# privacy-scaling-explorations/zkevm-specs

Hardware: AMD Instinct MI355X
Metric: BN254 constraint-rows/sec (higher is better)
Workload: dtype u256 (BN254 Fr: 4xu64 canonical cells, u32-limb Montgomery); 1 GPU; EVM circuit, 2^18 execution steps per GPU, mixed-opcode synthetic trace (BASELINE configs[2]); RW table 816377 rows, bytecode table 43913 rows; steps_per_gpu=262144, rw_rows=816377, bytecode_rows=43913, witness_copies=3

## Files before the change

### zkevm_specs_amd/csrc/evm_circuit.hpp

```cpp
#pragma once
#include "common.hpp"
#include "evm_tables.h"
#include "keccak.hpp"
#include "secp_constants.h"
#include "bigz.hpp"

enum { S_STATE = 0, S_RWC, S_CALL_ID, S_IS_ROOT, S_IS_CREATE, S_CH_LO, S_CH_HI, S_PC, S_SP, S_GAS, S_MWS, S_REV, S_LOG, STEP_NCELLS };
enum { R_RWC = 0, R_RW, R_TAG, R_ID, R_ADDR, R_FT, R_KEY_LO, R_KEY_HI, R_VAL_LO, R_VAL_HI, R_PREV_LO, R_PREV_HI, R_AUX_LO, R_AUX_HI, RW_NCELLS };
enum { B_HASH_LO = 0, B_HASH_HI, B_TAG, B_INDEX, B_IS_CODE, B_VALUE, BYTECODE_NCELLS };
enum { TX_NCELLS = 5, BLOCK_NCELLS = 4 };
enum { CT_IS_FIRST = 0, CT_SRC_ID_LO, CT_SRC_ID_HI, CT_SRC_TAG, CT_DST_ID_LO, CT_DST_ID_HI, CT_DST_TAG, CT_SRC_ADDR,
       CT_SRC_ADDR_END, CT_DST_ADDR, CT_LENGTH, CT_RLC_ACC, CT_RWC, CT_RWC_INC, COPY_T_NCELLS };
enum { XT_IS_STEP = 0, XT_ID, XT_IS_LAST, XT_BASE0, XT_BASE1, XT_BASE2, XT_BASE3, XT_EXP_LO, XT_EXP_HI, XT_RES_LO, XT_RES_HI,
       EXP_T_NCELLS };
enum { SIG_T_NCELLS = 9, ECC_T_NCELLS = 13 };
enum { AUX_PAIR = 3, AUX_ECRECOVER = 5, AUX_ECADD = 6, AUX_ECMUL = 7, AUX_ECPAIRING = 8 };
enum { CDT_Bytecode = 1, CDT_Memory, CDT_TxCalldata, CDT_TxLog, CDT_RlcAcc };

struct EvmDyn {
    u32 rw_sparse;
    u32 codes_n;
    u64 rw_base;
    u32 codes_mask;
    u32 agg_max_txs, agg_total_txs, agg_invalid_txs, agg_bad_invalid_rows, agg_total_wds;
    u32 dir_entries;
    u32 n_deferred;
    u32 agg_rw_dups;
};

struct EvmArgs {
    const EvmDyn* dyn;
    const u64* steps;
    const u32* step_recs;
    u64 n_steps;
    ZkTable rw, bytecode, tx, block;
    ZkTable copy, keccak, exp;
    ZkTable sig, ecc;
    ZkTable withdrawals;
    u32 agg_max_txs, agg_total_txs, agg_invalid_txs, agg_bad_invalid_rows, agg_total_wds;
    u32 agg_rw_dups;
    const u64* aux;
    const u32* aux_kind;
    u32 aux_cells;
    u32 rw_dense;
    u64 rw_base;
    const u64* rw_keys;
    ZkCodeDir codes;
    unsigned long long* prof;
    u32* defer_list;
    u32* defer_count;
    const u32* perm;
    u32 n_pairs;
    u32 opts;
    u32* defer_count_twin;
};

ZK_HD void evm_args_resolve(EvmArgs& a) {
#ifdef EVM_RESOLVE_OFF
    return;
#endif
    if (a.dyn) {
        const EvmDyn d = *a.dyn;
        a.rw_dense = (a.rw.n != 0u && d.rw_sparse == 0u) ? 1u : 0u;
        a.rw_base = d.rw_base;
        a.codes.n = d.codes_n;
        a.codes.mask = d.codes_mask;
        a.agg_max_txs = d.agg_max_txs; a.agg_total_txs = d.agg_total_txs; a.agg_invalid_txs = d.agg_invalid_txs;
        a.agg_bad_invalid_rows = d.agg_bad_invalid_rows; a.agg_total_wds = d.agg_total_wds;
        a.agg_rw_dups = d.agg_rw_dups;
    }
}

#ifndef EVM_HOT_BLOCK
#define EVM_HOT_BLOCK 128
#endif
#define EVM_STAGE_LANES EVM_HOT_BLOCK
#define EV_PROF_WAVE ((blockIdx.x * blockDim.x + threadIdx.x) >> 6)
#define EV_PROF_ON(a) ((a).prof && (threadIdx.x & 63) == 0 && EV_PROF_WAVE < 4096u)
#define EVM_STAGE_STRIDE (EVM_STAGE_LANES + 1)
#define EVM_STAGE_ENTRIES 40
#define EVM_STAGE_GAS 10
ZK_HD constexpr int evm_stage_entry(int s, int c) {
    return c == S_CH_LO || c == S_CH_HI ? 24 + s * 8 + (c - S_CH_LO) * 4
           : s * 12 + (c < S_CH_LO ? c : c == S_PC ? 5 : c == S_SP ? 6 : c == S_MWS ? 7 : c == S_REV ? 8 : c == S_LOG ? 9 : EVM_STAGE_GAS);
}
#define EVM_DIR_MAX_SLOTS 128
#define EVM_DIR_MAX_ENTRIES 32
#define EVM_DIR_SLOT_U64 (EVM_DIR_MAX_SLOTS / 2)
#define EVM_DIR_LDS_U64 (EVM_DIR_SLOT_U64 + EVM_DIR_MAX_ENTRIES * 12)
#if defined(ZK_HOSTSIM)
typedef const u64* EVM_LDS_PTR;
typedef const u32* EVM_LDS32_PTR;
#else
typedef const __attribute__((address_space(3))) u64* EVM_LDS_PTR;
typedef const __attribute__((address_space(3))) u32* EVM_LDS32_PTR;
#endif

struct Word {
    Fr lo, hi;
};
struct WordOrValue {
    Word w;
    bool is_word;
};

#ifndef EVM_FAST
#define EVM_FAST 0
#endif
struct Ins {
    const EvmArgs* a;
    u32 defer;
    u64 idx;
    u32 err;
    u32 seq;
    u64 rw_off;
    u32 pc_off;
    int sp_off;
    Fr rwc, call_id, sp, pc;
    u32 code_state, code_header_row, code_byte_base, code_n_bytes, code_header_ok;
    u64 code_header_value;
    EVM_LDS32_PTR stage;
    EVM_LDS_PTR dir_lds;
    u32 pre_op;
    bool pre_op_ok;
    u32 op_info, op_info_byte;
};

#if defined(ZK_HOSTSIM)
#define EV_PROF(I, k) do { } while (0)
#else
#define EV_PROF(I, k) do { if (EV_PROF_ON(*(I).a)) (I).a->prof[EV_PROF_WAVE * 8 + (k)] = __builtin_readcyclecounter(); } while (0)
#endif

ZK_HD void ev_fail(Ins& I, u32 kind) {
    if (I.err == 0u) I.err = ZK_CODE(kind, I.seq);
}
ZK_HD void ev_require(Ins& I, bool cond, u32 kind = ZK_ASSERT) {
    I.seq++;
    const u32 take = (cond ? 0u : 1u) & (I.err == 0u ? 1u : 0u);
    I.err = take ? ZK_CODE(kind, I.seq) : I.err;
}
#define EV_TRY(stmt) do { stmt; if (I.err) return; } while (0)
#define EV_TRYV(stmt, ret) do { stmt; if (I.err) return ret; } while (0)

ZK_HD Fr ev_step_cell(const EvmArgs& a, u64 step, int c) { return fr_load(a.steps + (step * STEP_NCELLS + c) * 4); }
ZK_HD Fr ev_staged_cell(const Ins& I, int s, int c) {
    Fr r = fr_zero();
    const int e = evm_stage_entry(s, c);
    const int n = (c == S_CH_LO || c == S_CH_HI) ? 4 : c == S_GAS ? 2 : 1;
#pragma unroll
    for (int w = 0; w < n; w++) r.v[w] = I.stage[(e + w) * EVM_STAGE_STRIDE];
    return r;
// ... 4326 lines not shown
```

### zkevm_specs_amd/csrc/evm_kernel.hpp

```cpp
#pragma once
#include "kernels.hpp"

#ifndef ZK_HOT_OCC
#define ZK_HOT_OCC 2
#endif
template <int G, int OCC, int BLOCK>
__global__ __launch_bounds__(BLOCK, OCC) void evm_steps_kernel(EvmArgs a, const u32* group_start, u32* status, ZkTally* tally) {
    u32 perm_t = 0;
    if (G == EVM_GROUP_ALL && a.perm) perm_t = a.perm[(u64)blockIdx.x * blockDim.x + threadIdx.x];
    if (G == EVM_GROUP_ALL && a.defer_count_twin != nullptr) {
        if (blockIdx.x == 0 && threadIdx.x == 0) *a.defer_count_twin = 0u;
        tally_clear_twin(tally);
    }
    __shared__ u64 s_dir[G == EVM_GROUP_ALL ? EVM_DIR_LDS_U64 : 1];
    const bool have_dir = G == EVM_GROUP_ALL && a.dyn != nullptr && a.codes.slots != nullptr && a.codes.entries != nullptr;
    if (have_dir) {
        for (u32 k = threadIdx.x; k < EVM_DIR_SLOT_U64; k += blockDim.x) s_dir[k] = (u64)a.codes.slots[2 * k] | ((u64)a.codes.slots[2 * k + 1] << 32);
        const u64* e = (const u64*)a.codes.entries;
        for (u32 k = threadIdx.x; k < EVM_DIR_MAX_ENTRIES * 12u; k += blockDim.x) s_dir[EVM_DIR_SLOT_U64 + k] = e[k];
    }
    evm_args_resolve(a);
    u32 lo = 0, hi = a.n_pairs;
    if (a.perm) {
        if (G == EVM_GROUP_ALL) hi = group_start[EVM_GROUP_WARM];
        else { lo = group_start[G]; hi = group_start[G + 1]; }
    }
    u64 t = (u64)lo + (u64)blockIdx.x * blockDim.x + threadIdx.x;
    const bool staged_launch = G == EVM_GROUP_ALL || (G == EVM_GROUP_WARM && BLOCK == EVM_HOT_BLOCK && a.perm != nullptr);
    __shared__ u32 s_stage[(G == EVM_GROUP_ALL || (G == EVM_GROUP_WARM && BLOCK == EVM_HOT_BLOCK)) ? EVM_STAGE_ENTRIES * EVM_STAGE_STRIDE : 1];
    if (staged_launch) {
      for (u32 vblock = blockIdx.x;; vblock += gridDim.x) {
        t = (u64)lo + (u64)vblock * blockDim.x + threadIdx.x;
        if ((u64)lo + (u64)vblock * blockDim.x >= (u64)hi) return;
        if (G != EVM_GROUP_ALL && vblock != blockIdx.x) __syncthreads();
        if (G != EVM_GROUP_ALL) perm_t = t < (u64)hi ? a.perm[t] : 0u;
        if (G == EVM_GROUP_ALL && EV_PROF_ON(a)) {
            a.prof[EV_PROF_WAVE * 8 + 5] = __builtin_readcyclecounter();
            a.prof[EV_PROF_WAVE * 8 + 6] = __builtin_amdgcn_s_memrealtime();
        }
        const bool dir_in_lds = have_dir && a.codes.n != 0 && a.codes.n <= EVM_DIR_MAX_ENTRIES && a.codes.mask < EVM_DIR_MAX_SLOTS;
        u32 code = 0;
        u64 idx = t;
        if (t < (u64)hi && a.perm) idx = perm_t;
        const bool mine = t < (u64)hi && idx != (u64)EVM_NO_PAIR;
        __attribute__((address_space(3))) u32* my = (__attribute__((address_space(3))) u32*)s_stage + threadIdx.x;
        const bool wide = a.step_recs ? evm_stage_steps_quad(a, (u32)idx, mine, my - (threadIdx.x & 63u))
                                      : evm_stage_steps_rows_quad(a, (u32)idx, mine, my - (threadIdx.x & 63u));
        if (dir_in_lds) __syncthreads();
        if (mine) {
#if EVM_FAST
            code = wide ? (u32)ZK_DEFERRED_BASE + 8u
                        : evm_check_step<G>(a, idx, (EVM_LDS32_PTR)my, dir_in_lds ? (EVM_LDS_PTR)(__attribute__((address_space(3))) u64*)s_dir : (EVM_LDS_PTR) nullptr);
            if (code >= ZK_DEFERRED_BASE && code != ZK_NOT_MINE) {
#ifdef ZK_DEFER_DEBUG
                if (a.prof) atomicAdd(&a.prof[4095 * 8 - 16 + (code & 15u)], 1ull);
#endif
                a.defer_list[atomicAdd(a.defer_count, 1u)] = (u32)idx;
                code = 0;
            } else
#else
#ifdef ZK_WARM_TWICE
            if (G == EVM_GROUP_WARM)
                code = evm_check_step<G>(a, idx, wide ? (EVM_LDS32_PTR) nullptr : (EVM_LDS32_PTR)my, (EVM_LDS_PTR) nullptr);
#endif
            code = evm_check_step<G>(a, idx, wide ? (EVM_LDS32_PTR) nullptr : (EVM_LDS32_PTR)my,
                                     dir_in_lds ? (EVM_LDS_PTR)(__attribute__((address_space(3))) u64*)s_dir : (EVM_LDS_PTR) nullptr);
#endif
            if (code == ZK_NOT_MINE) code = 0;
            else if (status) status[idx] = code;
        }
        tally_commit(tally, idx, code);
        if (G == EVM_GROUP_ALL && EV_PROF_ON(a)) a.prof[EV_PROF_WAVE * 8 + 7] = __builtin_amdgcn_s_memrealtime();
        if (G == EVM_GROUP_ALL) return;
      }
    } else {
        const u64 stride = (u64)gridDim.x * blockDim.x;
        for (; t < (u64)hi; t += stride) {
            const u64 idx = a.perm ? (u64)a.perm[t] : t;
            u32 code = idx == (u64)EVM_NO_PAIR ? (u32)ZK_NOT_MINE : evm_check_step<G>(a, idx);
            if (code == ZK_NOT_MINE) code = 0;
            else if (status) status[idx] = code;
            tally_commit(tally, idx, code);
        }
    }
}

#if defined(EVM_DEFERRED_KERNEL)
__global__ __launch_bounds__(256, 1) void evm_deferred_kernel(EvmArgs a, u32* status, ZkTally* tally) {
    evm_args_resolve(a);
    const u32 n_def = *a.defer_count;
    const u64 stride = (u64)gridDim.x * blockDim.x;
    for (u64 k = (u64)blockIdx.x * blockDim.x + threadIdx.x; k < (u64)n_def; k += stride) {
        const u64 idx = a.defer_list[k];
        u32 code = evm_check_step<EVM_GROUP_ALL>(a, idx);
        if (code == ZK_NOT_MINE) code = 0;
        else if (status) status[idx] = code;
        tally_commit(tally, idx, code);
    }
}
#endif
```

### zkevm_specs_amd/csrc/zkevm_hip.hip

```cpp
#include <hip/hip_runtime.h>
#include <hip/hip_ext.h>
#include <stdio.h>
#include <string.h>
#include <stdlib.h>
#include <chrono>
#include <string>
#include <vector>

#include <atomic>
#include <mutex>
#include <dlfcn.h>

#include "../../include/zkevm_hip.h"
#include "kernels.hpp"
#include "dist_tally.hpp"
#include "host_index.hpp"
#include "code_dir_build.hpp"

#define ZK_MAX_DEVICES 64
#define ZK_ECDSA_CHUNK_LANES (1ull << 17)
static std::mutex g_dev_mutex;
static hipStream_t g_own_stream[ZK_MAX_DEVICES] = {nullptr};
static hipStream_t g_batch_stream[ZK_MAX_DEVICES][2] = {{nullptr}};
static hipStream_t g_side_stream[ZK_MAX_DEVICES] = {nullptr};
// ... 110 lines not shown
__global__ void tally_reset_kernel(ZkTally* t, u32* counter = nullptr) {
    t[threadIdx.x].fail_count = 0ull;
    t[threadIdx.x].first_fail = ~0ull;
    if (counter && threadIdx.x == 0) *counter = 0u;
}


__global__ void slots_fill_kernel(u32* slots, u32 n) {
    u32 i = blockIdx.x * blockDim.x + threadIdx.x;
    if (i < n) slots[i] = ZK_EMPTY_SLOT;
}

template <u64 (*HASH)(const ZkTable&, u32)>
__global__ void index_build_kernel(ZkTable t, u32* slots, const ZkRwMeta* unless_dense = nullptr) {
    u32 r = blockIdx.x * blockDim.x + threadIdx.x;
    if (r >= t.n || (unless_dense && unless_dense->dense)) return;
    u32 s = (u32)HASH(t, r) & t.mask;
    while (atomicCAS(&slots[s], ZK_EMPTY_SLOT, r) != ZK_EMPTY_SLOT) s = (s + 1) & t.mask;
}
__global__ void slots_fill_unless_dense_kernel(u32* slots, u32 n, const ZkRwMeta* unless_dense) {
    u32 i = blockIdx.x * blockDim.x + threadIdx.x;
    if (i < n && !unless_dense->dense) slots[i] = ZK_EMPTY_SLOT;
}
__global__ void mpt_index_build_kernel(ZkTable t, u32* slots) {
    u32 r = blockIdx.x * blockDim.x + threadIdx.x;
    if (r >= t.n) return;
    const u64 h = state_mpt_key_hash(t, r);
    u32 s = (u32)h & t.mask;
    const u32 v = state_mpt_slot_value(t, r, h);
    while (atomicCAS(&slots[s], ZK_EMPTY_SLOT, v) != ZK_EMPTY_SLOT) s = (s + 1) & t.mask;
}
__global__ void rw_dense_check_kernel(ZkTable t, ZkRwMeta* meta) {
    const u32 r = blockIdx.x * blockDim.x + threadIdx.x;
    if (r >= t.n) return;
    const u64* p = t.cells + (u64)r * RW_NCELLS * 4;
    const u64* p0 = t.cells;
    const u64 base = p0[0];
    const bool ok = (p0[1] | p0[2] | p0[3]) == 0 && (p[1] | p[2] | p[3]) == 0 && p[0] == base + r && base + r >= base;
    if (r == 0) meta->base = base;
    if (!ok) atomicAnd(&meta->dense, 0u);
}

struct EvmSortArgs {
    const u64* steps;
    u32 n_pairs;
    u32* hist;
    u32* hist_next;
    u32* taken;
    uint16_t* bin16;
    u32* group_start;
    u32* perm;
    ZkTally* tally;
    u32* defer_count;
    u32* early_host;
    u32 early_seq;
};
#define EVM_EARLY_WORD 36u
__device__ __forceinline__ void evm_state_hist_body(u32 vblock, const u64* steps, u32 n_pairs, u32* hist, u32* taken, uint16_t* bin16, ZkTally* tally,
                                                    u32* defer_count) {
    __shared__ u32 local[EVM_N_BINS];
    if (vblock == 0) {
        if (threadIdx.x == 0 && defer_count) *defer_count = 0u;
        if (threadIdx.x == 0) {
            tally->fail_count = 0ull;
            tally->first_fail = ~0ull;
        }
        for (u32 k = threadIdx.x; k < EVM_N_BINS; k += blockDim.x) taken[k] = 0;
    }
    for (u32 k = threadIdx.x; k < EVM_N_BINS; k += blockDim.x) local[k] = 0;
    __syncthreads();
    u32 i = vblock * blockDim.x + threadIdx.x;
    if (i < n_pairs) {
        const u32 bin = evm_state_bin((u32)steps[((u64)i * STEP_NCELLS + S_STATE) * 4]);
        bin16[i] = (uint16_t)bin;
        atomicAdd(&local[bin], 1u);
    }
    __syncthreads();
    for (u32 k = threadIdx.x; k < EVM_N_BINS; k += blockDim.x)
        if (local[k]) atomicAdd(&hist[k], local[k]);
}
__global__ void evm_state_hist_kernel(const u64* steps, u32 n_pairs, u32* hist, u32* taken, uint16_t* bin16, ZkTally* tally, u32* defer_count) {
    evm_state_hist_body(blockIdx.x, steps, n_pairs, hist, taken, bin16, tally, defer_count);
}
__device__ __forceinline__ void evm_state_scatter_body(u32 vblock, const uint16_t* bin16, u32 n_pairs, const u32* hist, u32* hist_next,
                                                       u32* taken, u32* group_start, u32* perm, u32* early_host = nullptr, u32 early_seq = 0u) {
    __shared__ u32 sa[EVM_N_BINS], sb[EVM_N_BINS];
    __shared__ u32 local[EVM_N_BINS];
    __shared__ u32 base[EVM_N_BINS];
    __shared__ u32 gsh[EVM_N_GROUPS + 1];
    const u32 k = threadIdx.x;
    u32 c = 0, c_real = 0;
    if (k < EVM_N_BINS) {
        c_real = hist[k];
        c = k < (u32)EVM_GROUP_WARM * 128u ? ((c_real + 63u) & ~63u) : c_real;
        sa[k] = c;
        local[k] = 0;
        if (vblock == 0) hist_next[k] = 0;
    }
    __syncthreads();
    u32* src = sa;
    u32* dst = sb;
    for (u32 off = 1; off < EVM_N_BINS; off <<= 1) {
        if (k < EVM_N_BINS) dst[k] = src[k] + (k >= off ? src[k - off] : 0u);
        __syncthreads();
        u32* t = src; src = dst; dst = t;
    }
    u32 excl = 0;
    if (k < EVM_N_BINS) {
        excl = src[k] - c;
        if (vblock == 0) {
            if ((k & 127u) == 0) group_start[k >> 7] = gsh[k >> 7] = excl;
            if (k == EVM_N_BINS - 1) group_start[EVM_N_GROUPS] = gsh[EVM_N_GROUPS] = src[k];
            for (u32 j = c_real; j < c; j++) perm[excl + j] = EVM_NO_PAIR;
        }
    }
    const u32 i = vblock * blockDim.x + threadIdx.x;
    u32 bin = 0, rank = 0;
    if (i < n_pairs) {
        bin = bin16[i];
        rank = atomicAdd(&local[bin], 1u);
    }
    __syncthreads();
    if (vblock == 0 && k == 0 && early_host) {
        __hip_atomic_store(&early_host[EVM_EARLY_WORD], gsh[EVM_GROUP_WARM + 1] - gsh[EVM_GROUP_WARM], __ATOMIC_RELAXED, __HIP_MEMORY_SCOPE_SYSTEM);
        __hip_atomic_store(&early_host[EVM_EARLY_WORD + 1], gsh[EVM_GROUP_COLD + 1] - gsh[EVM_GROUP_COLD], __ATOMIC_RELAXED, __HIP_MEMORY_SCOPE_SYSTEM);
        __threadfence_system();
        __hip_atomic_store(&early_host[EVM_EARLY_WORD + 2], early_seq, __ATOMIC_RELEASE, __HIP_MEMORY_SCOPE_SYSTEM);
    }
    if (k < EVM_N_BINS && local[k]) base[k] = excl + atomicAdd(&taken[k], local[k]);
    __syncthreads();
    if (i < n_pairs) perm[base[bin] + rank] = i;
}
__global__ __launch_bounds__(1024) void evm_state_scatter_kernel(const uint16_t* bin16, u32 n_pairs, const u32* hist, u32* hist_next,
                                                                 u32* taken, u32* group_start, u32* perm) {
    evm_state_scatter_body(blockIdx.x, bin16, n_pairs, hist, hist_next, taken, group_start, perm);
}
__global__ __launch_bounds__(256) void evm_open_fill_kernel(uint4* ff, u64 n_ff, uint4* zero, u64 n_zero) {
    const u64 stride = (u64)gridDim.x * blockDim.x;
    const uint4 F = make_uint4(~0u, ~0u, ~0u, ~0u), Z = make_uint4(0u, 0u, 0u, 0u);
    for (u64 i = (u64)blockIdx.x * blockDim.x + threadIdx.x; i < n_ff; i += stride) ff[i] = F;
    for (u64 i = (u64)blockIdx.x * blockDim.x + threadIdx.x; i < n_zero; i += stride) zero[i] = Z;
}
__device__ __forceinline__ void rw_prepare_quad(const ZkTable& t, u64* keys, EvmDyn* dyn, u32 vthread) {
    const u32 r = vthread >> 2, q = vthread & 3u;
    const bool in = r < t.n;
    uint4 c0 = make_uint4(0, 0, 0, 0), c1 = c0, c2 = c0;
    u64 base = 0;
    u32 flags = 3u;
    if (in) {
        const uint4* p = reinterpret_cast<const uint4*>(t.cells + (u64)r * RW_NCELLS * 4) + q;
        c0 = p[0];
        c1 = p[4];
        c2 = p[8];
        if (q == 0) {
            base = t.cells[0];
            if (t.flags) flags = t.flags[r];
        }
    }
    bool fit, dense_ok;
    u64 w0 = 0, w1 = 0, w2 = 0, w3 = 0;
    const bool z0hi = (c0.y | c0.z | c0.w) == 0u, z1hi = (c1.y | c1.z | c1.w) == 0u, z2hi = (c2.y | c2.z | c2.w) == 0u;
    const bool z0 = z0hi && c0.x == 0u, z1 = z1hi && c1.x == 0u, z2 = z2hi && c2.x == 0u;
    if (q == 0) {
        const u64 rwc = (u64)c0.x | ((u64)c0.y << 32);
        dense_ok = (c0.z | c0.w) == 0u && rwc == base + r && base + r >= base;
        fit = z1hi && c1.x <= 255u;
        w0 = (u64)(c1.x & 0xffu) << 8 | ((u64)(flags & 3u) << 56) | (1ull << 63);
        w2 = (u64)c2.x | ((u64)c2.y << 32);
        w3 = (u64)c2.z | ((u64)c2.w << 32);
    } else if (q == 1) {
        dense_ok = z0;
        fit = z1 && z2hi;
        w0 = (u64)c2.x << 24;
    } else if (q == 2) {
        dense_ok = true;
        fit = z0hi && c0.x <= 255u && (c1.z | c1.w) == 0u && z2hi && c2.x <= 255u;
        w0 = (u64)(c0.x & 0xffu) | ((u64)(c2.x & 0xffu) << 16);
        w1 = (u64)c1.x | ((u64)c1.y << 32);
    } else {
        dense_ok = true;
        fit = z0 && z1 && z2;
    }
    const u32 qshift = threadIdx.x & 60u;
    const bool fits = ((__ballot(fit) >> qshift) & 0xfull) == 0xfull;
    const unsigned long long nd = __ballot(in && !dense_ok);
    if (nd != 0ull && (threadIdx.x & 63u) == 0) atomicOr(&dyn->rw_sparse, 1u);
    if (r == 0 && q == 0 && in) dyn->rw_base = base;
#pragma unroll
    for (int m = 1; m <= 2; m <<= 1) {
        w0 |= __shfl_xor(w0, m);
        w1 |= __shfl_xor(w1, m);
        w2 |= __shfl_xor(w2, m);
        w3 |= __shfl_xor(w3, m);
    }
    if (!fits) w0 = w1 = w2 = w3 = 0;
    if (in && q < 2) {
        const u64 a = q == 0 ? w0 : w2, b2 = q == 0 ? w1 : w3;
        reinterpret_cast<uint4*>(keys + (u64)r * 4)[q] = make_uint4((u32)a, (u32)(a >> 32), (u32)b2, (u32)(b2 >> 32));
    }
}
#define EVM_OPEN_TABLES 8
struct EvmOpenTables {
    ZkTable t[EVM_OPEN_TABLES];
    u32 block_start[EVM_OPEN_TABLES + 2];
    const u64* wds;
    u32 n_wds;
    EvmDyn* dyn;
    ZkTally* tally;
    ZkTable rw;
    u64* rw_keys;
    u32 dir_block0, rw_block0;
    DirBuild dir;
    const u64* steps;
    u32 n_steps;
// ... 404 lines not shown
    s->tally_last = s->d_tally;
    rc = dev_alloc(s, (void**)&s->d_status, (size_t)s->n * sizeof(u32));
    if (rc) return rc;
    HIP_TRY(hipMemsetAsync(s->d_status, 0, (size_t)s->n * sizeof(u32), s->stream));
    return 0;
}

extern "C" int zk_close(zk_session* s) {
    if (!s) return 0;
    (void)hipSetDevice(s->device);
    if (!s->stream_drained) (void)hipStreamSynchronize(s->stream);
    for (size_t k = 0; k < s->owned.size(); k++) arena_give(s->device, s->owned[k], s->owned_class[k]);
    {
        DevArena& A = g_arena[s->device];
        std::lock_guard<std::mutex> lock(A.m);
        for (hipEvent_t e : s->ev) A.events.push_back(e);
        if (s->ev_open0) A.events.push_back(s->ev_open0);
        if (s->ev_open1) A.events.push_back(s->ev_open1);
        if (s->ev_fork) A.events.push_back(s->ev_fork);
        if (s->ev_join) A.events.push_back(s->ev_join);
        if (s->h_result) A.pinned.push_back(s->h_result);
    }
    delete s;
    return 0;
}

extern "C" int zk_state_open(const uint64_t* rows, const uint32_t* flags, uint64_t n, const uint64_t* mpt,
                             uint64_t n_mpt, uint32_t opts, zk_session** out) {
    ARG_TRY(t_device >= 0, "zk_state_open: call zk_init first");
    HIP_TRY(hipSetDevice(t_device));
    ARG_TRY(out && rows && n > 0 && n < (1ull << 32), "zk_state_open: bad arguments");
    ARG_TRY(n_mpt < (1ull << 31), "zk_state_open: MPT table too large");
    const bool dev = opts & ZK_OPT_DEVICE_PTRS;
    const bool compact = opts & ZK_OPT_STATE_COMPACT;
    zk_session* s = new zk_session();
    s->kind = SESSION_STATE;
    s->n = n;
    int rc = 0;
    const void* p = nullptr;
    if ((rc = stage(s, rows, (size_t)n * (compact ? 15 : ST_NCELLS) * 32, dev, &p))) goto fail;
    s->state.rows.cells = (const u64*)p;
    s->state.rows.skip = compact ? 42u : 0u;
    if ((rc = stage(s, flags, (size_t)n * 4, dev, &p))) goto fail;
    s->state.rows.flags = (const u32*)p;
    s->state.rows.n = n;
    s->state.eval_lo = 0;
    s->state.eval_hi = n;
    if ((rc = stage(s, mpt, (size_t)n_mpt * MPT_NCELLS * 32, dev, &p))) goto fail;
    s->state.mpt.cells = (const u64*)p;
    s->state.mpt.flags = nullptr;
    s->state.mpt.n = (u32)n_mpt;
    s->state.mpt.ncells = MPT_NCELLS;
    if ((rc = build_index<state_mpt_key_hash>(s, s->state.mpt, true))) goto fail;
    if ((rc = session_common_init(s))) goto fail;
    *out = s;
    return 0;
fail:
    zk_close(s);
    return rc;
}

static int table_stage(zk_session* s, ZkTable& t, const uint64_t* cells, const uint32_t* flags, uint64_t n,
                       u32 ncells, bool dev) {
    const void* p = nullptr;
    int rc;
    if ((rc = stage(s, cells, (size_t)n * ncells * 32, dev, &p))) return rc;
    t.cells = (const u64*)p;
    if ((rc = stage(s, flags, (size_t)n * 4, dev, &p))) return rc;
    t.flags = (n && flags) ? (const u32*)p : nullptr;
    t.n = (u32)n;
    t.ncells = ncells;
    return 0;
}

#ifndef ZK_HIST_BLOCK
#define ZK_HIST_BLOCK 1024
#endif
static int evm_build_perm(zk_session* s) {
    const u32 n = s->evm.n_pairs;
    u32* h_cur = (s->evm_pass & 1u) ? s->d_hist2 : s->d_hist;
    u32* h_next = (s->evm_pass & 1u) ? s->d_hist : s->d_hist2;
    s->evm_pass++;
    hipLaunchKernelGGL(evm_state_hist_kernel, dim3((n + ZK_HIST_BLOCK - 1) / ZK_HIST_BLOCK), dim3(ZK_HIST_BLOCK), 0, s->stream, s->evm.steps, n, h_cur, s->d_cursor, s->d_bin16, s->d_tally, s->evm.defer_count);
    hipLaunchKernelGGL(evm_state_scatter_kernel, dim3((n + 1023) / 1024), dim3(1024), 0, s->stream, s->d_bin16, n, h_cur, h_next, s->d_cursor,
                       s->d_group_start, s->d_perm);
    HIP_TRY(hipGetLastError());
    return 0;
}

static inline u32 index_cap(u64 n) {
    u32 cap = 16;
    while (cap < 2 * n + 2) cap <<= 1;
    return cap;
}

extern "C" int zk_evm_open(const zk_evm_tables* t, uint32_t opts, zk_session** out) {
    ARG_TRY(t_device >= 0, "zk_evm_open: call zk_init first");
    HIP_TRY(hipSetDevice(t_device));
    ARG_TRY(t && out && t->steps && t->n_steps >= 2 && t->n_steps < (1ull << 32), "zk_evm_open: bad arguments");
    ARG_TRY(t->n_rw < (1ull << 31) && t->n_bytecode < (1ull << 31) && t->n_tx < (1ull << 31) && t->n_block < (1ull << 31) &&
            t->n_copy < (1ull << 31) && t->n_keccak < (1ull << 31) && t->n_exp < (1ull << 31) && t->n_withdrawals < (1ull << 31) &&
            t->n_sig < (1ull << 31) && t->n_ecc < (1ull << 31),
            "zk_evm_open: table too large");
    ARG_TRY(t->aux_cells == 0 || (t->aux_cells >= 2 && t->aux_cells <= 64), "zk_evm_open: aux_cells must be 0 (= 2) or 2..64");
    const bool dev = opts & ZK_OPT_DEVICE_PTRS;
    const bool generic = opts & ZK_OPT_GENERIC_INDEX;
    zk_session* s = new zk_session();
    s->kind = SESSION_EVM;
    s->n = t->n_steps - 1;
    s->side_stream = (opts & ZK_OPT_SIDE_STREAM) != 0;
    int rc = 0;
    const void* p = nullptr;
    EvmArgs& E = s->evm;
    if ((rc = stage(s, t->steps, (size_t)t->n_steps * STEP_NCELLS * 32, dev, &p))) goto fail;
    E.steps = (const u64*)p;
    E.n_steps = t->n_steps;
    E.n_pairs = (u32)(t->n_steps - 1);
    if ((rc = table_stage(s, E.rw, t->rw, t->rw_flags, t->n_rw, RW_NCELLS, dev))) goto fail;
    if ((rc = table_stage(s, E.bytecode, t->bytecode, nullptr, t->n_bytecode, BYTECODE_NCELLS, dev))) goto fail;
    if ((rc = table_stage(s, E.tx, t->tx, t->tx_flags, t->n_tx, TX_NCELLS, dev))) goto fail;
    if ((rc = table_stage(s, E.block, t->block, t->block_flags, t->n_block, BLOCK_NCELLS, dev))) goto fail;
    if ((rc = table_stage(s, E.copy, t->copy, nullptr, t->n_copy, COPY_T_NCELLS, dev))) goto fail;
    if ((rc = table_stage(s, E.keccak, t->keccak, nullptr, t->n_keccak, KECCAK_NCELLS, dev))) goto fail;
    if ((rc = table_stage(s, E.exp, t->exp, nullptr, t->n_exp, EXP_T_NCELLS, dev))) goto fail;
    if ((rc = table_stage(s, E.sig, t->sig, nullptr, t->n_sig, SIG_T_NCELLS, dev))) goto fail;
    if ((rc = table_stage(s, E.ecc, t->ecc, nullptr, t->n_ecc, ECC_T_NCELLS, dev))) goto fail;
    if ((rc = table_stage(s, E.withdrawals, t->withdrawals, nullptr, t->n_withdrawals, 4, dev))) goto fail;
    E.withdrawals.slots = nullptr;
    E.withdrawals.mask = 0;
    E.aux = nullptr;
    E.aux_kind = nullptr;
    E.aux_cells = t->aux_cells ? t->aux_cells : 2u;
    if (t->aux && t->aux_kind) {
        if ((rc = stage(s, t->aux, (size_t)t->n_steps * E.aux_cells * 32, dev, &p))) goto fail;
        E.aux = (const u64*)p;
        if ((rc = stage(s, t->aux_kind, (size_t)t->n_steps * 4, dev, &p))) goto fail;
        E.aux_kind = (const u32*)p;
    }
    {
        ZkTable* const small[EVM_OPEN_TABLES] = {&E.tx, &E.block, &E.bytecode, &E.copy, &E.keccak, &E.exp, &E.sig, &E.ecc};
        const bool want_dir = !generic && t->n_bytecode != 0;
        size_t n_ff = 0;
        u32 caps[EVM_OPEN_TABLES];
        for (int k = 0; k < EVM_OPEN_TABLES; k++) { caps[k] = index_cap(small[k]->n); n_ff += caps[k]; }
        const u32 cap_rw = index_cap(E.rw.n), cap_big = want_dir ? index_cap(t->n_bytecode) : 0u;
        n_ff += (size_t)cap_rw + 2 * (size_t)cap_big + (want_dir ? DIRB_SMALL_SLOTS : 0u);
        u32* ff = nullptr;
        if ((rc = dev_alloc(s, (void**)&ff, n_ff * sizeof(u32)))) goto fail;
        u32* cur = ff;
        for (int k = 0; k < EVM_OPEN_TABLES; k++) { small[k]->slots = cur; small[k]->mask = caps[k] - 1; cur += caps[k]; }
        E.rw.slots = cur; E.rw.mask = cap_rw - 1; cur += cap_rw;
        u32* const dir_rep = cur; cur += cap_big;
        u32* const dir_first = cur; cur += cap_big;
        u32* const small_slots = cur;
        const size_t dyn_bytes = 256, hist_bytes = EVM_N_BINS * sizeof(u32), status_bytes = (((size_t)s->n * sizeof(u32)) + 15) & ~(size_t)15;
        const size_t zero_bytes = dyn_bytes + 2 * hist_bytes + status_bytes + 3 * (size_t)cap_big * 4;
        char* zero = nullptr;
        if ((rc = dev_alloc(s, (void**)&zero, zero_bytes))) goto fail;
        EvmResultBlock* const rb = (EvmResultBlock*)zero;
        EvmDyn* dyn = &rb->dyn;
        s->d_result = rb;
        if ((rc = arena_pinned(s->device, &s->h_result))) goto fail;
        {
            void* hd = nullptr;
            if (hipHostGetDevicePointer(&hd, s->h_result, 0) == hipSuccess) s->h_result_dev = (u32*)hd;
            (void)hipGetLastError();
        }
// ... 7 lines not shown
        E.defer_count = &dyn->n_deferred;
        if ((rc = dev_alloc(s, (void**)&E.defer_list, (size_t)E.n_pairs * sizeof(u32)))) goto fail;
        s->d_tally = rb->tally;
        s->tally_last = s->d_tally;
        {
            const u64 n16 = n_ff / 4 + zero_bytes / 16;
            const u32 fill_grid = (u32)(n16 / 256 < 2048 ? (n16 + 255) / 256 : 2048);
            if (arena_event(s->device, &s->ev_open0) || arena_event(s->device, &s->ev_open1)) s->ev_open0 = s->ev_open1 = nullptr;
            hipExtLaunchKernelGGL(evm_open_fill_kernel, dim3(fill_grid ? fill_grid : 1u), dim3(256), 0, s->stream, s->ev_open0, nullptr, 0, (uint4*)ff,
                                  (u64)(n_ff / 4), (uint4*)zero, (u64)(zero_bytes / 16));
        }
        E.rw_dense = 0;
        E.rw_base = 0;
        E.rw_keys = nullptr;
        E.codes.n = 0;
        E.codes.mask = 0;
        E.codes.packed = nullptr;
        E.codes.entries = nullptr;
        E.codes.slots = nullptr;
        E.agg_max_txs = E.agg_total_txs = E.agg_invalid_txs = E.agg_bad_invalid_rows = E.agg_total_wds = E.agg_rw_dups = 0;
        EvmOpenTables o;
        memset(&o, 0, sizeof o);
        u32 blk = 0;
        for (int k = 0; k < EVM_OPEN_TABLES; k++) { o.t[k] = *small[k]; o.block_start[k] = blk; blk += (small[k]->n + 255u) / 256u; }
        o.block_start[EVM_OPEN_TABLES] = blk;
        blk += (u32)((t->n_withdrawals + 255) / 256);
        o.block_start[EVM_OPEN_TABLES + 1] = blk;
        o.wds = E.withdrawals.cells;
        o.n_wds = (u32)t->n_withdrawals;
        o.dyn = dyn;
        o.tally = s->d_tally;
        o.rw = E.rw;
        if (t->n_rw && !generic) {
            u64* d_keys = nullptr;
            if ((rc = dev_alloc(s, (void**)&d_keys, (size_t)t->n_rw * 32))) goto fail;
            E.rw_keys = d_keys;
            o.rw_keys = d_keys;
        }
        const u32 rw_row_blocks = o.rw_keys ? (u32)((t->n_rw + 63) / 64) : 0u;
        o.dir_block0 = blk;
        u32 dir_row_blocks = 0;
        if (want_dir) {
            DirBuild& d = o.dir;
            d.rows = E.bytecode.cells;
            d.n = (u32)t->n_bytecode;
            d.rep = dir_rep;
            d.first = dir_first;
            d.last = dir_last;
            d.runs = dir_last + cap_big;
            d.bad = dir_last + 2 * (size_t)cap_big;
            d.big_mask = cap_big - 1;
            d.small_slots = small_slots;
            d.dyn = dyn;
            if ((rc = dev_alloc(s, (void**)&d.packed, (size_t)d.n * sizeof(uint16_t)))) goto fail;
            if ((rc = dev_alloc(s, (void**)&d.entries, (size_t)DIRB_MAX_ENTRIES * sizeof(ZkCodeEntry)))) goto fail;
            if ((rc = dev_alloc(s, (void**)&d.list, (size_t)DIRB_MAX_ENTRIES * 4))) goto fail;
            dir_row_blocks = (d.n + 255u) / 256u;
            E.codes.entries = d.entries;
            E.codes.slots = d.small_slots;
            E.codes.packed = d.packed;
        }
        if ((rc = dev_alloc(s, (void**)&s->d_cursor, EVM_N_BINS * sizeof(u32)))) goto fail;
        if ((rc = dev_alloc(s, (void**)&s->d_bin16, (size_t)E.n_pairs * sizeof(uint16_t)))) goto fail;
        s->d_group_start = rb->group_start;
        if ((rc = dev_alloc(s, (void**)&s->d_perm, ((size_t)E.n_pairs + EVM_PERM_PAD + 2 * EVM_HOT_BLOCK) * sizeof(u32)))) goto fail;
        const bool sorted = !(opts & ZK_OPT_NO_STATE_SORT);
        o.hist_block0 = o.dir_block0 + dir_row_blocks;
        u32 hist_blocks = 0, scatter_blocks = 0;
        if (sorted) {
            o.sort.steps = E.steps; o.sort.n_pairs = E.n_pairs; o.sort.hist = s->d_hist; o.sort.hist_next = s->d_hist2;
            o.sort.taken = s->d_cursor; o.sort.bin16 = s->d_bin16; o.sort.group_start = s->d_group_start; o.sort.perm = s->d_perm;
            o.sort.tally = s->d_tally;
            o.sort.defer_count = E.defer_count;
            if ((opts & ZK_OPT_SINGLE_PASS) && s->h_result_dev && evm_lazy_tail_enabled() && !(opts & ZK_OPT_SIDE_STREAM)) {
                static std::atomic<u32> g_early_seq{0};
                u32 q = ++g_early_seq;
                if (!q) q = ++g_early_seq;
                __atomic_store_n(&((u32*)s->h_result)[EVM_EARLY_WORD + 2], 0u, __ATOMIC_RELEASE);
                s->early_seq = q;
                o.sort.early_host = s->h_result_dev;
                o.sort.early_seq = q;
            }
            hist_blocks = (E.n_pairs + 255u) / 256u;
            scatter_blocks = (E.n_pairs + EVM_OPEN_P2_BLOCK - 1u) / EVM_OPEN_P2_BLOCK;
            s->evm_pass = 1;
            s->perm_ready = true;
        }
        o.rw_block0 = o.hist_block0 + hist_blocks;
        o.rec_block0 = o.rw_block0 + rw_row_blocks;
        u32 rec_blocks = 0;
        E.step_recs = nullptr;
        if (!(opts & ZK_OPT_SINGLE_PASS)) {
            u32* recs = nullptr;
            if ((rc = dev_alloc(s, (void**)&recs, (size_t)t->n_steps * EVM_REC_WORDS * sizeof(u32)))) goto fail;
            o.steps = E.steps; o.n_steps = (u32)t->n_steps; o.step_recs = recs;
            E.step_recs = recs;
            rec_blocks = (u32)((t->n_steps + 63) / 64);
        }
        const u32 grid1 = o.rec_block0 + rec_blocks;
        {
            static const u32 spread = [] { const char* e = getenv("ZK_P1_LAT_SPREAD"); const int v = e ? atoi(e) : 2; return (u32)(v < 0 ? 0 : v); }();
            o.lat_period = (o.rw_block0 && spread) ? o.rec_block0 / (spread * o.rw_block0) : 0u;
        }
#ifdef ZK_DIAG_P1
        if (const char* e = getenv("ZK_DIAG_P1_SKIP")) o.diag_skip = (u32)atoi(e);
#endif
        {
            const u32 dir_blocks = want_dir ? DIRB_MAX_ENTRIES / EVM_OPEN_P2_BLOCK : 0u;
            const u32 rw_blocks = t->n_rw ? EVM_OPEN_RW_GENERIC_BLOCKS : 0u;
            bool phase2 = scatter_blocks + dir_blocks + rw_blocks != 0;
#ifdef ZK_DIAG_P1
            if (o.diag_skip) phase2 = false;
#endif
            hipExtLaunchKernelGGL(evm_open_phase1_kernel, dim3(grid1 ? grid1 : 1u), dim3(256), 0, s->stream, nullptr, phase2 ? nullptr : s->ev_open1, 0, o);
            if (phase2)
                hipExtLaunchKernelGGL(evm_open_phase2_kernel, dim3(scatter_blocks + dir_blocks + rw_blocks), dim3(EVM_OPEN_P2_BLOCK), 0, s->stream, nullptr,
                                      s->ev_open1, 0, o, scatter_blocks, dir_blocks, generic ? 1u : 0u);
        }
        if (hipGetLastError() != hipSuccess) { rc = -2; g_err = "zk_evm_open: a build kernel failed to launch"; goto fail; }
    }
    E.opts = (t->begin_with_first_step ? 1u : 0u) | (t->end_with_last_step ? 2u : 0u);
    E.prof = nullptr;
    if (getenv("ZK_EVM_PROF")) {
        if ((rc = dev_alloc(s, (void**)&E.prof, 1024 * 4 * 8 * sizeof(unsigned long long)))) goto fail;
        if (hipMemsetAsync(E.prof, 0, 1024 * 4 * 8 * sizeof(unsigned long long), s->stream) != hipSuccess) { rc = -2; goto fail; }
    }
    E.perm = (opts & ZK_OPT_NO_STATE_SORT) ? nullptr : s->d_perm;
    *out = s;
    return 0;
fail:
    zk_close(s);
    return rc;
}

static void session_timing(zk_session* s, double pass_ms, double* open_ms, double* span_ms);
static int evm_enqueue_tail(zk_session* s);
static bool evm_publish_enqueue(zk_session* s);
extern "C" int zk_evm_verify(const zk_evm_tables* t, uint32_t opts, uint32_t* status_out, zk_result* result) {
    ARG_TRY(result, "zk_evm_verify: result is null");
    zk_session* s = nullptr;
    const auto h0 = std::chrono::steady_clock::now();
    int rc = zk_evm_open(t, opts | ZK_OPT_SINGLE_PASS, &s);
    if (rc) return rc;
    const auto h1 = std::chrono::steady_clock::now();
    const bool dev = opts & ZK_OPT_DEVICE_PTRS;
    rc = zk_launch(s, (dev && status_out) ? status_out : nullptr);
    const auto h2 = std::chrono::steady_clock::now();
    if (!rc) rc = zk_collect(s, result);
    const auto h3 = std::chrono::steady_clock::now();
    if (!rc) {
        t_timing[1] = result->kernel_ms;
        session_timing(s, result->kernel_ms, &t_timing[0], &t_timing[2]);
        for (int k = 0; k < 3; k++) t_timing_sum[k] += t_timing[k];
        t_timing_count++;
    }
    if (!rc && status_out && !dev) rc = zk_read_status(s, status_out);
    zk_close(s);
    const auto h4 = std::chrono::steady_clock::now();
    t_host_phase[0] = std::chrono::duration<double, std::micro>(h1 - h0).count();
    t_host_phase[1] = std::chrono::duration<double, std::micro>(h2 - h1).count();
    t_host_phase[2] = std::chrono::duration<double, std::micro>(h3 - h2).count();
    t_host_phase[3] = std::chrono::duration<double, std::micro>(h4 - h3).count();
    return rc;
}

extern "C" int zk_evm_verify_batch(const zk_evm_tables* const* t, uint64_t n, uint32_t opts, zk_result* results) {
    ARG_TRY(t_device >= 0, "zk_evm_verify_batch: call zk_init first");
// ... 2768 lines not shown
```

Baseline: 1.595 billion rows/s.

## Prefetch directory via async LDS loads, speculative staging, warp-scan scatter

The steps kernel now copies the code directory into LDS with asynchronous global_load_lds 16-byte requests instead of per-thread loads and stores. It also reads the EvmDyn parameters and group bounds up front and starts staging step rows before the hot-range exit check, so those loads overlap with the rest of setup. The state scatter kernel replaces the LDS ping-pong prefix scan, which needed many barriers, with wavefront shuffle scans. It adds one dedicated owner block that writes group_start, the NO_PAIR padding and the early host words, so the other blocks skip that serial work. The cost is one extra scatter block and speculative staging loads for threads beyond the hot range.

Result: no change. 1.585 billion rows/s (-0.6%).

```diff
diff --git a/zkevm_specs_amd/csrc/evm_circuit.hpp b/zkevm_specs_amd/csrc/evm_circuit.hpp
--- a/zkevm_specs_amd/csrc/evm_circuit.hpp
+++ b/zkevm_specs_amd/csrc/evm_circuit.hpp
@@ -55,19 +55,22 @@
     u32* defer_count_twin;
 };
 
+ZK_HD void evm_args_patch(EvmArgs& a, const EvmDyn& d) {
+    a.rw_dense = (a.rw.n != 0u && d.rw_sparse == 0u) ? 1u : 0u;
+    a.rw_base = d.rw_base;
+    a.codes.n = d.codes_n;
+    a.codes.mask = d.codes_mask;
+    a.agg_max_txs = d.agg_max_txs; a.agg_total_txs = d.agg_total_txs; a.agg_invalid_txs = d.agg_invalid_txs;
+    a.agg_bad_invalid_rows = d.agg_bad_invalid_rows; a.agg_total_wds = d.agg_total_wds;
+    a.agg_rw_dups = d.agg_rw_dups;
+}
 ZK_HD void evm_args_resolve(EvmArgs& a) {
 #ifdef EVM_RESOLVE_OFF
     return;
 #endif
     if (a.dyn) {
         const EvmDyn d = *a.dyn;
-        a.rw_dense = (a.rw.n != 0u && d.rw_sparse == 0u) ? 1u : 0u;
-        a.rw_base = d.rw_base;
-        a.codes.n = d.codes_n;
-        a.codes.mask = d.codes_mask;
-        a.agg_max_txs = d.agg_max_txs; a.agg_total_txs = d.agg_total_txs; a.agg_invalid_txs = d.agg_invalid_txs;
-        a.agg_bad_invalid_rows = d.agg_bad_invalid_rows; a.agg_total_wds = d.agg_total_wds;
-        a.agg_rw_dups = d.agg_rw_dups;
+        evm_args_patch(a, d);
     }
 }
 
diff --git a/zkevm_specs_amd/csrc/evm_kernel.hpp b/zkevm_specs_amd/csrc/evm_kernel.hpp
--- a/zkevm_specs_amd/csrc/evm_kernel.hpp
+++ b/zkevm_specs_amd/csrc/evm_kernel.hpp
@@ -4,26 +4,44 @@
 #ifndef ZK_HOT_OCC
 #define ZK_HOT_OCC 2
 #endif
+template <int BLOCK>
+__device__ __forceinline__ void evm_dir_mirror_request(const ZkCodeDir& codes, u64* s_dir) {
+    constexpr u32 n_chunks = EVM_DIR_LDS_U64 / 2u, slot_chunks = EVM_DIR_SLOT_U64 / 2u;
+    static_assert(EVM_DIR_LDS_U64 % 2 == 0 && EVM_DIR_SLOT_U64 % 2 == 0 && BLOCK % 64 == 0, "the directory mirror is copied in 16-byte chunks, 64 per wavefront");
+    const u32 wave0 = (u32)__builtin_amdgcn_readfirstlane((int)(threadIdx.x & ~63u));
+#pragma unroll
+    for (u32 j = 0; j < (n_chunks + BLOCK - 1) / BLOCK; j++) {
+        const u32 c = j * BLOCK + threadIdx.x;
+        const char* src = c < slot_chunks ? (const char*)codes.slots + 16u * c : (const char*)codes.entries + 16u * (c - slot_chunks);
+        if (c < n_chunks)
+            __builtin_amdgcn_global_load_lds((const __attribute__((address_space(1))) void*)src,
+                                             (__attribute__((address_space(3))) void*)((__attribute__((address_space(3))) char*)s_dir + 16u * (j * BLOCK + wave0)), 16, 0, 0);
+    }
+}
 template <int G, int OCC, int BLOCK>
 __global__ __launch_bounds__(BLOCK, OCC) void evm_steps_kernel(EvmArgs a, const u32* group_start, u32* status, ZkTally* tally) {
-    u32 perm_t = 0;
-    if (G == EVM_GROUP_ALL && a.perm) perm_t = a.perm[(u64)blockIdx.x * blockDim.x + threadIdx.x];
+    u32 perm_t = 0, lo = 0, hi = a.n_pairs;
+    const bool have_dir = G == EVM_GROUP_ALL && a.dyn != nullptr && a.codes.slots != nullptr && a.codes.entries != nullptr;
+    __shared__ __attribute__((aligned(16))) u64 s_dir[G == EVM_GROUP_ALL ? EVM_DIR_LDS_U64 : 1];
+    if (G == EVM_GROUP_ALL && a.perm != nullptr && a.dyn != nullptr) {
+        perm_t = a.perm[(u64)blockIdx.x * BLOCK + threadIdx.x];
+        if (have_dir) evm_dir_mirror_request<BLOCK>(a.codes, s_dir);
+        const u32 hot_end = group_start[EVM_GROUP_WARM];
+        const EvmDyn d = *a.dyn;
+        hi = hot_end;
+        evm_args_patch(a, d);
+    } else {
+        if (G == EVM_GROUP_ALL && a.perm) perm_t = a.perm[(u64)blockIdx.x * BLOCK + threadIdx.x];
+        if (have_dir) evm_dir_mirror_request<BLOCK>(a.codes, s_dir);
+        evm_args_resolve(a);
+        if (a.perm) {
+            if (G == EVM_GROUP_ALL) hi = group_start[EVM_GROUP_WARM];
+            else { lo = group_start[G]; hi = group_start[G + 1]; }
+        }
+    }
     if (G == EVM_GROUP_ALL && a.defer_count_twin != nullptr) {
         if (blockIdx.x == 0 && threadIdx.x == 0) *a.defer_count_twin = 0u;
         tally_clear_twin(tally);
-    }
-    __shared__ u64 s_dir[G == EVM_GROUP_ALL ? EVM_DIR_LDS_U64 : 1];
-    const bool have_dir = G == EVM_GROUP_ALL && a.dyn != nullptr && a.codes.slots != nullptr && a.codes.entries != nullptr;
-    if (have_dir) {
-        for (u32 k = threadIdx.x; k < EVM_DIR_SLOT_U64; k += blockDim.x) s_dir[k] = (u64)a.codes.slots[2 * k] | ((u64)a.codes.slots[2 * k + 1] << 32);
-        const u64* e = (const u64*)a.codes.entries;
-        for (u32 k = threadIdx.x; k < EVM_DIR_MAX_ENTRIES * 12u; k += blockDim.x) s_dir[EVM_DIR_SLOT_U64 + k] = e[k];
-    }
-    evm_args_resolve(a);
-    u32 lo = 0, hi = a.n_pairs;
-    if (a.perm) {
-        if (G == EVM_GROUP_ALL) hi = group_start[EVM_GROUP_WARM];
-        else { lo = group_start[G]; hi = group_start[G + 1]; }
     }
     u64 t = (u64)lo + (u64)blockIdx.x * blockDim.x + threadIdx.x;
     const bool staged_launch = G == EVM_GROUP_ALL || (G == EVM_GROUP_WARM && BLOCK == EVM_HOT_BLOCK && a.perm != nullptr);
@@ -31,21 +49,27 @@
     if (staged_launch) {
       for (u32 vblock = blockIdx.x;; vblock += gridDim.x) {
         t = (u64)lo + (u64)vblock * blockDim.x + threadIdx.x;
-        if ((u64)lo + (u64)vblock * blockDim.x >= (u64)hi) return;
+        if (G != EVM_GROUP_ALL && (u64)lo + (u64)vblock * blockDim.x >= (u64)hi) return;
         if (G != EVM_GROUP_ALL && vblock != blockIdx.x) __syncthreads();
         if (G != EVM_GROUP_ALL) perm_t = t < (u64)hi ? a.perm[t] : 0u;
         if (G == EVM_GROUP_ALL && EV_PROF_ON(a)) {
             a.prof[EV_PROF_WAVE * 8 + 5] = __builtin_readcyclecounter();
             a.prof[EV_PROF_WAVE * 8 + 6] = __builtin_amdgcn_s_memrealtime();
         }
-        const bool dir_in_lds = have_dir && a.codes.n != 0 && a.codes.n <= EVM_DIR_MAX_ENTRIES && a.codes.mask < EVM_DIR_MAX_SLOTS;
         u32 code = 0;
         u64 idx = t;
-        if (t < (u64)hi && a.perm) idx = perm_t;
+        if (a.perm && (G == EVM_GROUP_ALL || t < (u64)hi)) idx = perm_t;
+        const bool stageable = G == EVM_GROUP_ALL ? idx < (u64)a.n_pairs : (t < (u64)hi && idx != (u64)EVM_NO_PAIR);
+        __attribute__((address_space(3))) u32* my = (__attribute__((address_space(3))) u32*)s_stage + threadIdx.x;
+        const bool wide = a.step_recs ? evm_stage_steps_quad(a, (u32)idx, stageable, my - (threadIdx.x & 63u))
+                                      : evm_stage_steps_rows_quad(a, (u32)idx, stageable, my - (threadIdx.x & 63u));
+        if (G == EVM_GROUP_ALL && (u64)blockIdx.x * BLOCK >= (u64)hi) {
+            __builtin_amdgcn_s_waitcnt(0);
+            return;
+        }
+        if (t >= (u64)hi) idx = t;
         const bool mine = t < (u64)hi && idx != (u64)EVM_NO_PAIR;
-        __attribute__((address_space(3))) u32* my = (__attribute__((address_space(3))) u32*)s_stage + threadIdx.x;
-        const bool wide = a.step_recs ? evm_stage_steps_quad(a, (u32)idx, mine, my - (threadIdx.x & 63u))
-                                      : evm_stage_steps_rows_quad(a, (u32)idx, mine, my - (threadIdx.x & 63u));
+        const bool dir_in_lds = have_dir && a.codes.n != 0 && a.codes.n <= EVM_DIR_MAX_ENTRIES && a.codes.mask < EVM_DIR_MAX_SLOTS;
         if (dir_in_lds) __syncthreads();
         if (mine) {
 #if EVM_FAST
diff --git a/zkevm_specs_amd/csrc/zkevm_hip.hip b/zkevm_specs_amd/csrc/zkevm_hip.hip
--- a/zkevm_specs_amd/csrc/zkevm_hip.hip
+++ b/zkevm_specs_amd/csrc/zkevm_hip.hip
@@ -216,54 +216,62 @@
 __global__ void evm_state_hist_kernel(const u64* steps, u32 n_pairs, u32* hist, u32* taken, uint16_t* bin16, ZkTally* tally, u32* defer_count) {
     evm_state_hist_body(blockIdx.x, steps, n_pairs, hist, taken, bin16, tally, defer_count);
 }
+#define EVM_SCATTER_BLOCKS(n_pairs, block) (((n_pairs) + (block) - 1u) / (block) + 1u)
 __device__ __forceinline__ void evm_state_scatter_body(u32 vblock, const uint16_t* bin16, u32 n_pairs, const u32* hist, u32* hist_next,
                                                        u32* taken, u32* group_start, u32* perm, u32* early_host = nullptr, u32 early_seq = 0u) {
-    __shared__ u32 sa[EVM_N_BINS], sb[EVM_N_BINS];
+    static_assert(EVM_N_BINS % 64 == 0 && (EVM_N_GROUPS * 128) == EVM_N_BINS, "a group is 128 bins = two wavefronts of the scan");
+    __shared__ u32 wsum[EVM_N_BINS / 64];
     __shared__ u32 local[EVM_N_BINS];
     __shared__ u32 base[EVM_N_BINS];
     __shared__ u32 gsh[EVM_N_GROUPS + 1];
     const u32 k = threadIdx.x;
-    u32 c = 0, c_real = 0;
+    const bool owner = vblock == 0;
+    const u32 i = (vblock - 1u) * blockDim.x + threadIdx.x;
+    const bool has_pair = !owner && i < n_pairs;
+    const u32 c_real = k < EVM_N_BINS ? hist[k] : 0u;
+    const u32 bin = has_pair ? (u32)bin16[i] : 0u;
+    u32 c = 0, incl = 0;
     if (k < EVM_N_BINS) {
-        c_real = hist[k];
         c = k < (u32)EVM_GROUP_WARM * 128u ? ((c_real + 63u) & ~63u) : c_real;
-        sa[k] = c;
+        incl = c;
+        const u32 lane = k & 63u;
+#pragma unroll
+        for (u32 off = 1; off < 64u; off <<= 1) {
+            const u32 up = (u32)__shfl_up((int)incl, off);
+            if (lane >= off) incl += up;
+        }
+        if (lane == 63u) wsum[k >> 6] = incl;
         local[k] = 0;
-        if (vblock == 0) hist_next[k] = 0;
     }
     __syncthreads();
-    u32* src = sa;
-    u32* dst = sb;
-    for (u32 off = 1; off < EVM_N_BINS; off <<= 1) {
-        if (k < EVM_N_BINS) dst[k] = src[k] + (k >= off ? src[k - off] : 0u);
-        __syncthreads();
-        u32* t = src; src = dst; dst = t;
-    }
     u32 excl = 0;
     if (k < EVM_N_BINS) {
-        excl = src[k] - c;
-        if (vblock == 0) {
+        excl = incl - c;
+        for (u32 w = 0; w < (k >> 6); w++) excl += wsum[w];
+    }
+    if (owner) {
+        if (k < EVM_N_BINS) {
+            hist_next[k] = 0;
             if ((k & 127u) == 0) group_start[k >> 7] = gsh[k >> 7] = excl;
-            if (k == EVM_N_BINS - 1) group_start[EVM_N_GROUPS] = gsh[EVM_N_GROUPS] = src[k];
+            if (k == EVM_N_BINS - 1) group_start[EVM_N_GROUPS] = gsh[EVM_N_GROUPS] = excl + c;
+        }
+        __syncthreads();
+        if (k == 0 && early_host) {
+            __hip_atomic_store(&early_host[EVM_EARLY_WORD], gsh[EVM_GROUP_WARM + 1] - gsh[EVM_GROUP_WARM], __ATOMIC_RELAXED, __HIP_MEMORY_SCOPE_SYSTEM);
+            __hip_atomic_store(&early_host[EVM_EARLY_WORD + 1], gsh[EVM_GROUP_COLD + 1] - gsh[EVM_GROUP_COLD], __ATOMIC_RELAXED, __HIP_MEMORY_SCOPE_SYSTEM);
+            __threadfence_system();
+            __hip_atomic_store(&early_host[EVM_EARLY_WORD + 2], early_seq, __ATOMIC_RELEASE, __HIP_MEMORY_SCOPE_SYSTEM);
+        }
+        if (k < EVM_N_BINS)
             for (u32 j = c_real; j < c; j++) perm[excl + j] = EVM_NO_PAIR;
-        }
-    }
-    const u32 i = vblock * blockDim.x + threadIdx.x;
-    u32 bin = 0, rank = 0;
-    if (i < n_pairs) {
-        bin = bin16[i];
-        rank = atomicAdd(&local[bin], 1u);
-    }
+        return;
+    }
+    u32 rank = 0;
+    if (has_pair) rank = atomicAdd(&local[bin], 1u);
     __syncthreads();
-    if (vblock == 0 && k == 0 && early_host) {
-        __hip_atomic_store(&early_host[EVM_EARLY_WORD], gsh[EVM_GROUP_WARM + 1] - gsh[EVM_GROUP_WARM], __ATOMIC_RELAXED, __HIP_MEMORY_SCOPE_SYSTEM);
-        __hip_atomic_store(&early_host[EVM_EARLY_WORD + 1], gsh[EVM_GROUP_COLD + 1] - gsh[EVM_GROUP_COLD], __ATOMIC_RELAXED, __HIP_MEMORY_SCOPE_SYSTEM);
-        __threadfence_system();
-        __hip_atomic_store(&early_host[EVM_EARLY_WORD + 2], early_seq, __ATOMIC_RELEASE, __HIP_MEMORY_SCOPE_SYSTEM);
-    }
     if (k < EVM_N_BINS && local[k]) base[k] = excl + atomicAdd(&taken[k], local[k]);
     __syncthreads();
-    if (i < n_pairs) perm[base[bin] + rank] = i;
+    if (has_pair) perm[base[bin] + rank] = i;
 }
 __global__ __launch_bounds__(1024) void evm_state_scatter_kernel(const uint16_t* bin16, u32 n_pairs, const u32* hist, u32* hist_next,
                                                                  u32* taken, u32* group_start, u32* perm) {
@@ -834,7 +842,7 @@
     u32* h_next = (s->evm_pass & 1u) ? s->d_hist : s->d_hist2;
     s->evm_pass++;
     hipLaunchKernelGGL(evm_state_hist_kernel, dim3((n + ZK_HIST_BLOCK - 1) / ZK_HIST_BLOCK), dim3(ZK_HIST_BLOCK), 0, s->stream, s->evm.steps, n, h_cur, s->d_cursor, s->d_bin16, s->d_tally, s->evm.defer_count);
-    hipLaunchKernelGGL(evm_state_scatter_kernel, dim3((n + 1023) / 1024), dim3(1024), 0, s->stream, s->d_bin16, n, h_cur, h_next, s->d_cursor,
+    hipLaunchKernelGGL(evm_state_scatter_kernel, dim3(EVM_SCATTER_BLOCKS(n, 1024u)), dim3(1024), 0, s->stream, s->d_bin16, n, h_cur, h_next, s->d_cursor,
                        s->d_group_start, s->d_perm);
     HIP_TRY(hipGetLastError());
     return 0;
@@ -1008,7 +1016,7 @@
                 o.sort.early_seq = q;
             }
             hist_blocks = (E.n_pairs + 255u) / 256u;
-            scatter_blocks = (E.n_pairs + EVM_OPEN_P2_BLOCK - 1u) / EVM_OPEN_P2_BLOCK;
+            scatter_blocks = EVM_SCATTER_BLOCKS(E.n_pairs, EVM_OPEN_P2_BLOCK);
             s->evm_pass = 1;
             s->perm_ready = true;
         }
```
